# nagadomi/nunif

Hardware: NVIDIA H100
Metric: waifu2x_input_megapixels_per_sec (higher is better)
Workload: dtype f16

## Files before the change

nunif_b200/csrc/swin_attention_mma.cu:

```cuda
#include "common.cuh"
#include "gemm_wgmma.cuh"
#include "swin_kernels.h"
#include "tmap.h"

namespace nb200 {

extern int g_tune[16];

namespace {
constexpr int WS = 6, WTOK = 36, WPAD = 48, HEADS = 6;
constexpr const char* SHIFT_ONE_AXIS_MSG =
    "shifted window attention needs H and W both equal to the 6-token window or both larger (torchvision drops the shift per "
    "axis; these kernels shift both axes or neither)";
}

constexpr int NKT = 5;

template <int D>
struct AttnCtx {
    __half* sq;
    const int* sreg;
    const float4* bf;
    const __half* kbase[NKT];
    const __half* vbase[3];
    int hc, g, t4;
    float scale;
    bool boundary;
};

template <int D, int LD, bool LAST, int BNT = 6>
__device__ __forceinline__ void attn_mtile(const AttnCtx<D>& cx, int mt) {
    constexpr uint32_t ONES = 0x3C003C00u;
    constexpr int HL = LAST ? 1 : 2;
    const int g = cx.g, t4 = cx.t4, hc = cx.hc;
    const int row0 = min(mt * 16 + g, WTOK - 1), row1 = min(mt * 16 + g + 8, WTOK - 1);
    float s[NKT][4];
#pragma unroll
    for (int nt = 0; nt < NKT; ++nt)
#pragma unroll
        for (int r = 0; r < 4; ++r) s[nt][r] = 0.f;
#pragma unroll
    for (int kt = 0; kt < D / 16; ++kt) {
        uint32_t a[4];
        const __half* p0 = cx.sq + row0 * LD + hc + kt * 16 + 2 * t4;
        const __half* p1 = cx.sq + row1 * LD + hc + kt * 16 + 2 * t4;
        a[0] = *reinterpret_cast<const uint32_t*>(p0);
        a[1] = *reinterpret_cast<const uint32_t*>(p1);
        a[2] = *reinterpret_cast<const uint32_t*>(p0 + 8);
        a[3] = *reinterpret_cast<const uint32_t*>(p1 + 8);
#pragma unroll
        for (int nt = 0; nt < NKT; ++nt) {
            const __half* pk = cx.kbase[nt] + kt * 16;
            mma16816(s[nt], a, *reinterpret_cast<const uint32_t*>(pk), *reinterpret_cast<const uint32_t*>(pk + 8));
        }
    }
#pragma unroll
    for (int nt = 0; nt < NKT; ++nt) {
        const float4 bv = BNT == 6 ? __ldg(cx.bf + (mt * 6 + nt) * 32) : cx.bf[(mt * BNT + nt) * 32];
        s[nt][0] = fmaf(s[nt][0], cx.scale, bv.x);
        s[nt][1] = fmaf(s[nt][1], cx.scale, bv.y);
        if (!LAST) {
            s[nt][2] = fmaf(s[nt][2], cx.scale, bv.z);
            s[nt][3] = fmaf(s[nt][3], cx.scale, bv.w);
        }
    }
    if (cx.boundary) {
        const int q0 = cx.sreg[row0], q1 = cx.sreg[row1];
#pragma unroll
        for (int nt = 0; nt < NKT; ++nt)
#pragma unroll
            for (int e = 0; e < 2; ++e) {
                const int cr = cx.sreg[min(nt * 8 + 2 * t4 + e, WTOK - 1)];
                if (cr != q0) s[nt][e] += -100.0f * 1.4426950408889634f;
                if (!LAST && cr != q1) s[nt][2 + e] += -100.0f * 1.4426950408889634f;
            }
    }
#pragma unroll
    for (int hlf = 0; hlf < HL; ++hlf) {
        float mx = -1e30f;
#pragma unroll
        for (int nt = 0; nt < NKT; ++nt) mx = fmaxf(mx, fmaxf(s[nt][2 * hlf], s[nt][2 * hlf + 1]));
        mx = fmaxf(mx, __shfl_xor_sync(0xffffffffu, mx, 1));
        mx = fmaxf(mx, __shfl_xor_sync(0xffffffffu, mx, 2));
#pragma unroll
        for (int nt = 0; nt < NKT; ++nt)
#pragma unroll
            for (int e = 0; e < 2; ++e) {
                s[nt][2 * hlf + e] = ex2(s[nt][2 * hlf + e] - mx);
            }
    }
    if (LAST) {
#pragma unroll
        for (int nt = 0; nt < NKT; ++nt) s[nt][2] = s[nt][3] = 0.f;
    }
    float o[D / 8][4], osum[4] = {0.f, 0.f, 0.f, 0.f};
#pragma unroll
    for (int nt = 0; nt < D / 8; ++nt)
#pragma unroll
        for (int r = 0; r < 4; ++r) o[nt][r] = 0.f;
#pragma unroll
    for (int kt = 0; kt < 2; ++kt) {
        uint32_t a[4];
        a[0] = pack_half2(s[2 * kt][0], s[2 * kt][1]);
        a[1] = pack_half2(s[2 * kt][2], s[2 * kt][3]);
        a[2] = pack_half2(s[2 * kt + 1][0], s[2 * kt + 1][1]);
        a[3] = pack_half2(s[2 * kt + 1][2], s[2 * kt + 1][3]);
        mma16816(osum, a, ONES, ONES);
#pragma unroll
        for (int nt = 0; nt < D / 8; ++nt) {
            uint32_t b[2];
            ldmatrix_x2_trans(b, smem_u32(cx.vbase[kt] + nt * 8));
            mma16816(o[nt], a, b[0], b[1]);
        }
    }
    {
        const uint32_t a0 = pack_half2(s[4][0], s[4][1]), a1 = pack_half2(s[4][2], s[4][3]);
        mma1688(osum, a0, a1, ONES);
#pragma unroll
        for (int nt = 0; nt < D / 8; ++nt) {
            mma1688(o[nt], a0, a1, ldmatrix_x1_trans(smem_u32(cx.vbase[2] + nt * 8)));
        }
    }
    const float inv0 = __fdividef(1.f, osum[0]);
    const float inv1 = LAST ? 0.f : __fdividef(1.f, osum[2]);
    __syncwarp();
    const int r0 = mt * 16 + g, r1 = r0 + 8;
#pragma unroll
    for (int nt = 0; nt < D / 8; ++nt) {
        if (!LAST || r0 < WTOK) *reinterpret_cast<uint32_t*>(cx.sq + r0 * LD + hc + nt * 8 + 2 * t4) = pack_half2(o[nt][0] * inv0, o[nt][1] * inv0);
        if (!LAST) *reinterpret_cast<uint32_t*>(cx.sq + r1 * LD + hc + nt * 8 + 2 * t4) = pack_half2(o[nt][2] * inv1, o[nt][3] * inv1);
    }
}

template <int D>
__global__ void __launch_bounds__(192, D == 16 ? 6 : 4) window_attention_mma_kernel(const __half* __restrict__ qkv, const float4* __restrict__ bias_frag,
                                                                   __half* __restrict__ out, int H, int W, int shift,
                                                                   size_t plane) {
    if (threadIdx.x == 0) NB_PDL_TRIGGER();
    constexpr int C = D * HEADS;
    constexpr int LD = C + 8;
    extern __shared__ __align__(16) unsigned char smem_raw[];
    __half* sq = reinterpret_cast<__half*>(smem_raw);
    __half* sk = sq + WTOK * LD;
    __half* sv = sk + WTOK * LD;
    int* stok = reinterpret_cast<int*>(sv + WTOK * LD);
    int* sreg = stok + WTOK;
    const int nww = W / WS;
    const int wx = blockIdx.x % nww, wy = blockIdx.x / nww, b = blockIdx.y;
    const int tid = threadIdx.x;
    if (tid < WPAD) {
        int reg = -1;
        if (tid < WTOK) {
            const int ry = wy * WS + tid / WS, rx = wx * WS + tid % WS;
            const int y = (ry + shift) % H, x = (rx + shift) % W;
            stok[tid] = (b * H + y) * W + x;
            int hr = 0, wr = 0;
            if (shift > 0) {
                hr = ry < H - WS ? 0 : (ry < H - shift ? 1 : 2);
                wr = rx < W - WS ? 0 : (rx < W - shift ? 1 : 2);
            }
            reg = hr * 3 + wr;
        }
        sreg[tid] = reg;
    }
    __syncthreads();
    constexpr int VPT = C / 8;
    constexpr int RG = 192 / VPT;
    const int vv = tid % VPT, rg = tid / VPT;
    for (int t = rg; t < WTOK; t += RG) {
        const __half* src = qkv + (size_t)stok[t] * C + vv * 8;
        __half* dst = sq + t * LD + vv * 8;
        cp_async16(dst, src);
        cp_async16(dst + WTOK * LD, src + plane);
        cp_async16(dst + 2 * WTOK * LD, src + 2 * plane);
    }
    cp_async_commit();
    cp_async_wait<0>();
    __syncthreads();

    const int head = tid >> 5, lane = tid & 31, g = lane >> 2, t4 = lane & 3;
    const int hc = head * D;
    const float scale = ((D == 16) ? 0.25f : 0.17677669529663687f) * 1.4426950408889634f;
    const bool boundary = shift > 0 && (wy == gridDim.x / nww - 1 || wx == nww - 1);
    const float4* bf = bias_frag + (size_t)head * (3 * 6 * 32) + lane;
    AttnCtx<D> cx;
    cx.sq = sq; cx.sreg = sreg; cx.bf = bf; cx.hc = hc; cx.g = g; cx.t4 = t4; cx.scale = scale; cx.boundary = boundary;
#pragma unroll
    for (int nt = 0; nt < NKT; ++nt) cx.kbase[nt] = sk + min(nt * 8 + g, WTOK - 1) * LD + hc + 2 * t4;
    cx.vbase[0] = sv + (lane & 15) * LD + hc;
    cx.vbase[1] = sv + (16 + (lane & 15)) * LD + hc;
    cx.vbase[2] = sv + min(32 + (lane & 7), WTOK - 1) * LD + hc;
#pragma unroll 1
    for (int mt = 0; mt < 2; ++mt) attn_mtile<D, LD, false>(cx, mt);
    attn_mtile<D, LD, true>(cx, 2);
    __syncthreads();
    for (int t = rg; t < WTOK; t += RG)
        *reinterpret_cast<uint4*>(out + (size_t)stok[t] * C + vv * 8) = *reinterpret_cast<const uint4*>(sq + t * LD + vv * 8);
}

__global__ void build_bias_frag_kernel(const float* __restrict__ table, float4* __restrict__ frag) {
    const int i = blockIdx.x * blockDim.x + threadIdx.x;
    if (i >= HEADS * 3 * 6 * 32) return;
    const int lane = i & 31, nt = (i >> 5) % 6, mt = (i / (32 * 6)) % 3, head = i / (32 * 6 * 3);
    const int g = lane >> 2, t4 = lane & 3;
    float v[4];
#pragma unroll
    for (int r = 0; r < 4; ++r) {
        const int row = mt * 16 + g + 8 * (r >> 1), col = nt * 8 + 2 * t4 + (r & 1);
        if (col >= WTOK) v[r] = -1e30f;
        else if (row >= WTOK) v[r] = 0.f;
        else {
            const int qy = row / WS, qx = row % WS, ky = col / WS, kx = col % WS;
            v[r] = 1.4426950408889634f * table[((qy - ky + WS - 1) * (2 * WS - 1) + (qx - kx + WS - 1)) * HEADS + head];
        }
    }
    frag[i] = make_float4(v[0], v[1], v[2], v[3]);
}

int build_bias_frag(cudaStream_t st, const float* table, float* frag) {
    build_bias_frag_kernel<<<(HEADS * 3 * 6 * 32 + 255) / 256, 256, 0, st>>>(table, reinterpret_cast<float4*>(frag));
    NB_LAUNCHED();
    return 0;
}

template <int D>
static size_t attn_smem_bytes() {
    constexpr int C = D * HEADS, LD = C + 8;
    return (size_t)3 * WTOK * LD * 2 + (WTOK + WPAD) * 4 + 16;
}

static int check_window_geometry(const char* func, bool fused, int H, int W, int C, int* shift) {
    auto refuse = [&](const std::string& msg) { return fail(std::string(func) + ": " + msg); };
    if (H % WS != 0 || W % WS != 0) return refuse("feature map must be a multiple of the 6x6 window");
    if (C != 96 && C != 192) return refuse(std::string(fused ? "fused " : "") + "window attention supports C=96 (d=16) and C=192 (d=32)");
    if (*shift != 0 && (H == WS) != (W == WS)) return refuse(SHIFT_ONE_AXIS_MSG);
    if (WS >= H) *shift = 0;
    return 0;
}

int window_attention(cudaStream_t st, const __half* qkv, const float* bias_frag_f, __half* out, int B, int H, int W, int C,
                     int shift, size_t plane) {
    const float4* bias_table = reinterpret_cast<const float4*>(bias_frag_f);
    if (check_window_geometry(__func__, false, H, W, C, &shift)) return 1;
    dim3 grid((H / WS) * (W / WS), B);
    ProfScope ps(st, PC_ATTN, (double)B * H * W * C * 4 * 2, (double)B * H * W * C * 3 * 2, (double)B * H * W * C * 2);
    if (C == 96) {
        const int want = g_tune[6] > 0 ? g_tune[6] : 72;
        if (ensure_dyn_smem((const void*)window_attention_mma_kernel<16>, attn_smem_bytes<16>(), want)) return 1;
        window_attention_mma_kernel<16><<<grid, 192, attn_smem_bytes<16>(), st>>>(qkv, bias_table, out, H, W, shift, plane);
    } else {
        const int want = g_tune[6] > 0 ? g_tune[6] : 86;
        if (ensure_dyn_smem((const void*)window_attention_mma_kernel<32>, attn_smem_bytes<32>(), want)) return 1;
        window_attention_mma_kernel<32><<<grid, 192, attn_smem_bytes<32>(), st>>>(qkv, bias_table, out, H, W, shift, plane);
    }
    NB_LAUNCHED();
    return 0;
}


constexpr int FA_ROWS = 128, FA_WIN = 3, FA_SLOT = 96 * 64, FA_KPS = 3, FA_STAGES = 4;
constexpr int FA_MMA_THREADS = GEMM_CONSUMER_THREADS, FA_PRODUCER_WARP = FA_MMA_THREADS / 32, FA_ATTN_WARPS = 11;
constexpr int FA_THREADS = FA_MMA_THREADS + 32 + 32 * FA_ATTN_WARPS;
constexpr int FA_LD = 32 + 8;
constexpr int FA_CHUNK_BYTES = FA_WIN * 3 * WTOK * FA_LD * 2;
constexpr int FA_STAGE = FA_KPS * FA_SLOT;

template <int C>
struct FaCfg {
    static constexpr int X_BYTES = FA_ROWS * C * 2;
    static constexpr bool SBF = C == 96;
    static constexpr int SBF_BYTES = SBF ? HEADS * 3 * NKT * 32 * 16 : 0;
    static constexpr int SBF_OFF = 2 * X_BYTES + FA_STAGES * FA_STAGE + 2 * FA_CHUNK_BYTES + 4 * WPAD * 4 + (2 * FA_STAGES + 8) * 8 +
                                   3 * C * 4;
    static constexpr int SMEM = SBF_OFF + SBF_BYTES + 1024;
    static_assert(SBF_OFF % 16 == 0, "float4 bias fragments");
    static_assert(SMEM <= 232448, "over the 227 KB opt-in shared memory of an H100 CTA");
};

__device__ __forceinline__ int fa_token(int b, int wy, int wx, int t, int H, int W, int shift) {
    int y = wy * WS + t / WS + shift, xx = wx * WS + t % WS + shift;
    if (y >= H) y -= H;
    if (xx >= W) xx -= W;
    return (b * H + y) * W + xx;
}

template <int C>
__global__ void __launch_bounds__(FA_THREADS, 1) swin_attn_fused_kernel(const __grid_constant__ CUtensorMap wmap,
                                                                        const __half* __restrict__ x, const float* __restrict__ bqkv,
                                                                        const float4* __restrict__ bias_frag, __half* __restrict__ out,
                                                                        int H, int W, int shift, int nwin) {
    using Cfg = FaCfg<C>;
    constexpr int D = C / HEADS, KB = C / 32, NCH = C / 32, HPC = 32 / D;
    constexpr int IPC = 3 * FA_WIN * HPC, IPT = NCH * IPC;
    constexpr int SPC = KB / FA_KPS;
    constexpr int VPR = C / 8;
    static_assert(KB % FA_KPS == 0, "a ring stage holds FA_KPS K-blocks of one chunk");
    static_assert(FA_WIN == 3, "the gather selects among 3 windows");
    extern __shared__ uint8_t smem_dyn[];
    uint8_t* smem = smem_dyn + ((1024u - (smem_u32(smem_dyn) & 1023u)) & 1023u);
    uint8_t* sx = smem;
    uint8_t* ring = smem + 2 * Cfg::X_BYTES;
    __half* schunk = reinterpret_cast<__half*>(ring + FA_STAGES * FA_STAGE);
    int* sreg = reinterpret_cast<int*>(reinterpret_cast<uint8_t*>(schunk) + 2 * FA_CHUNK_BYTES);
    uint64_t* full = reinterpret_cast<uint64_t*>(sreg + 4 * WPAD);
    uint64_t* empty = full + FA_STAGES;
    uint64_t* afull = empty + FA_STAGES;
    uint64_t* aempty = afull + 2;
    uint64_t* cfull = aempty + 2;
    uint64_t* cempty = cfull + 2;
    float* sbias = reinterpret_cast<float*>(cempty + 2);
    float4* sbf = reinterpret_cast<float4*>(smem + Cfg::SBF_OFF);
    const int tid = threadIdx.x, warp = tid >> 5, lane = tid & 31;
    const int nww = W / WS, nwy = H / WS;
    const int ntiles = (nwin + FA_WIN - 1) / FA_WIN;
    const int ntl = (ntiles - (int)blockIdx.x + (int)gridDim.x - 1) / (int)gridDim.x;

    if (tid < 4 * WPAD) {
        const int p = tid / WPAD, t = tid % WPAD;
        int reg = -1;
        if (t < WTOK) {
            const int hr = (p & 2) ? (t / WS < WS - shift ? 1 : 2) : 0;
            const int wr = (p & 1) ? (t % WS < WS - shift ? 1 : 2) : 0;
            reg = hr * 3 + wr;
        }
        sreg[tid] = reg;
    }
    for (int i = tid; i < 3 * C; i += FA_THREADS) sbias[i] = bqkv[i];
    if (Cfg::SBF)
        for (int i = tid; i < HEADS * 3 * NKT * 32; i += FA_THREADS)
            sbf[i] = __ldg(bias_frag + ((i >> 5) / NKT * 6 + (i >> 5) % NKT) * 32 + (i & 31));
    for (int i = tid; i < 2 * (FA_ROWS - FA_WIN * WTOK) * VPR; i += FA_THREADS) {
        const int bsel = i / ((FA_ROWS - FA_WIN * WTOK) * VPR), j = i % ((FA_ROWS - FA_WIN * WTOK) * VPR);
        const int r = FA_WIN * WTOK + j / VPR, u = j % VPR;
        *reinterpret_cast<uint4*>(sx + bsel * Cfg::X_BYTES + (u >> 2) * (FA_ROWS * 64) + stage_off<32>(r, u & 3)) =
            make_uint4(0u, 0u, 0u, 0u);
    }
    if (tid == FA_MMA_THREADS) {
        tma_prefetch_desc(&wmap);
        for (int s = 0; s < FA_STAGES; ++s) {
            mbar_init(&full[s], 1);
            mbar_init(&empty[s], 2);
        }
        for (int b = 0; b < 2; ++b) {
            mbar_init(&afull[b], 32 * FA_ATTN_WARPS);
            mbar_init(&aempty[b], 2);
            mbar_init(&cfull[b], FA_MMA_THREADS / 32);
            mbar_init(&cempty[b], IPC);
        }
        fence_barrier_init();
    }
    fence_async_smem();
    __syncthreads();
    if (tid == 0) NB_PDL_TRIGGER();

    if (warp == FA_PRODUCER_WARP) {
        if (elect_one()) {
            int q = 0;
#pragma unroll 1
            for (int k = 0; k < ntl; ++k) {
#pragma unroll 1
                for (int i = 0; i < NCH * SPC; ++i, ++q) {
                    const int s = q % FA_STAGES, c = i / SPC, kb0 = (i % SPC) * FA_KPS;
                    mbar_wait(&empty[s], ((q / FA_STAGES) & 1) ^ 1);
                    mbar_expect_tx(&full[s], FA_STAGE);
#pragma unroll
                    for (int kk = 0; kk < FA_KPS; ++kk)
#pragma unroll
                        for (int m = 0; m < 3; ++m)
                            tma_load_2d(&wmap, &full[s], ring + s * FA_STAGE + kk * FA_SLOT + m * 32 * 64, (kb0 + kk) * 32, m * C + 32 * c);
                }
            }
        }
        return;
    }

    const float scale = ((D == 16) ? 0.25f : 0.17677669529663687f) * 1.4426950408889634f;
    const int g = lane >> 2, t4 = lane & 3;
    if (warp > FA_PRODUCER_WARP) {
        const int aw = warp - FA_PRODUCER_WARP - 1;
        auto gather = [&](int tile, uint8_t* sa) {
            int wb[FA_WIN], wwy[FA_WIN], wwx[FA_WIN];
#pragma unroll
            for (int w = 0; w < FA_WIN; ++w) {
                const int gw = tile * FA_WIN + w, b = gw / (nww * nwy), rw = gw - b * (nww * nwy);
                wb[w] = gw < nwin ? b : -1;
                wwy[w] = rw / nww;
                wwx[w] = rw - wwy[w] * nww;
            }
            for (int i = aw * 32 + lane; i < FA_WIN * WTOK * VPR; i += 32 * FA_ATTN_WARPS) {
                const int r = i / VPR, u = i % VPR, w = r / WTOK;
                const int b = w == 0 ? wb[0] : (w == 1 ? wb[1] : wb[2]);
                const int wy = w == 0 ? wwy[0] : (w == 1 ? wwy[1] : wwy[2]), wx = w == 0 ? wwx[0] : (w == 1 ? wwx[1] : wwx[2]);
                uint8_t* dst = sa + (u >> 2) * (FA_ROWS * 64) + stage_off<32>(r, u & 3);
                if (b >= 0) cp_async16(dst, x + (size_t)fa_token(b, wy, wx, r - w * WTOK, H, W, shift) * C + u * 8);
                else *reinterpret_cast<uint4*>(dst) = make_uint4(0u, 0u, 0u, 0u);
            }
            cp_async_commit();
        };
        auto gathered = [&](int kt) {
            cp_async_wait<0>();
            fence_async_smem();
            mbar_arrive(&afull[kt & 1]);
        };
        gather(blockIdx.x, sx);
        gathered(0);
        int kcur = -1, nth = 0;
#pragma unroll 1
        for (int n = aw; n < ntl * IPT; n += FA_ATTN_WARPS) {
            const int gc = n / IPC, item = n - gc * IPC, c = gc % NCH;
            const int kt = n / IPT, tile = blockIdx.x + kt * gridDim.x;
            mbar_wait(&cfull[gc & 1], (gc >> 1) & 1);
            if (kt != kcur) {
                kcur = kt;
                nth = 0;
            }
            if (kt + 1 < ntl && nth == 0) {
                mbar_wait(&aempty[(kt + 1) & 1], (((kt + 1) >> 1) & 1) ^ 1);
                gather(tile + gridDim.x, sx + ((kt + 1) & 1) * Cfg::X_BYTES);
            }
            if (kt + 1 < ntl && nth == 1) gathered(kt + 1);
            ++nth;
            const int mt = item / (FA_WIN * HPC), pr = item - mt * (FA_WIN * HPC), w = pr / HPC, hh = pr - w * HPC;
            const int gw = tile * FA_WIN + w;
            if (gw < nwin) {
                const int b = gw / (nww * nwy), r = gw % (nww * nwy), wy = r / nww, wx = r % nww, head = c * HPC + hh;
                const bool lrow = wy == nwy - 1, lcol = wx == nww - 1;
                __half* sq = schunk + (gc & 1) * (FA_CHUNK_BYTES / 2) + w * 3 * WTOK * FA_LD;
                __half* sk = sq + WTOK * FA_LD;
                __half* sv = sk + WTOK * FA_LD;
                AttnCtx<D> cx;
                cx.sq = sq; cx.sreg = sreg + (2 * lrow + lcol) * WPAD;
                cx.bf = Cfg::SBF ? sbf + head * (3 * NKT * 32) + lane : bias_frag + (size_t)head * (3 * 6 * 32) + lane;
                cx.hc = hh * D; cx.g = g; cx.t4 = t4; cx.scale = scale;
                cx.boundary = shift > 0 && (lrow || lcol);
#pragma unroll
                for (int nt = 0; nt < NKT; ++nt) cx.kbase[nt] = sk + min(nt * 8 + g, WTOK - 1) * FA_LD + cx.hc + 2 * t4;
                cx.vbase[0] = sv + (lane & 15) * FA_LD + cx.hc;
                cx.vbase[1] = sv + (16 + (lane & 15)) * FA_LD + cx.hc;
                cx.vbase[2] = sv + min(32 + (lane & 7), WTOK - 1) * FA_LD + cx.hc;
                constexpr int BNT = Cfg::SBF ? NKT : 6;
                if (mt < 2) attn_mtile<D, FA_LD, false, BNT>(cx, mt);
                else attn_mtile<D, FA_LD, true, BNT>(cx, 2);
                __syncwarp();
                const int nrow = mt < 2 ? 16 : WTOK - 32;
                for (int e = lane; e < nrow * (D / 8); e += 32) {
                    const int tk = 16 * mt + e / (D / 8), u = e % (D / 8);
                    *reinterpret_cast<uint4*>(out + (size_t)fa_token(b, wy, wx, tk, H, W, shift) * C + head * D + u * 8) =
                        *reinterpret_cast<const uint4*>(sq + tk * FA_LD + cx.hc + u * 8);
                }
            }
            __syncwarp();
            if (lane == 0) mbar_arrive(&cempty[gc & 1]);
        }
        return;
    }

    const int wg = tid >> 7, t = tid & 127;
    const int row0 = wg * 64 + (t >> 5) * 16 + ((t & 31) >> 2);
    const int cq = 2 * (t & 3);
    int q = 0, gc = 0;
#pragma unroll 1
    for (int k = 0; k < ntl; ++k) {
        mbar_wait(&afull[k & 1], (k >> 1) & 1);
        const uint32_t a_base = smem_u32(sx + (k & 1) * Cfg::X_BYTES) + wg * 64 * 64;
#pragma unroll 1
        for (int c = 0; c < NCH; ++c, ++gc) {
            float acc[48];
#pragma unroll
            for (int j = 0; j < 48; ++j) acc[j] = 0.f;
#pragma unroll 1
            for (int j = 0; j < SPC; ++j, ++q) {
                const int s = q % FA_STAGES;
                mbar_wait(&full[s], (q / FA_STAGES) & 1);
                wgmma_fence();
#pragma unroll
                for (int kk = 0; kk < FA_KPS; ++kk) {
                    const uint32_t a = a_base + (j * FA_KPS + kk) * (FA_ROWS * 64), bb = smem_u32(ring + s * FA_STAGE + kk * FA_SLOT);
                    wgmma_f16<96>(acc, make_kmajor_desc<64>(a), make_kmajor_desc<64>(bb), 1u);
                    wgmma_f16<96>(acc, make_kmajor_desc<64>(a + 32), make_kmajor_desc<64>(bb + 32), 1u);
                }
                wgmma_commit();
                wgmma_wait<1>();
                if (j > 0 && t == 0) mbar_arrive(&empty[(q - 1) % FA_STAGES]);
            }
            wgmma_wait<0>();
            if (t == 0) {
                mbar_arrive(&empty[(q - 1) % FA_STAGES]);
                if (c == NCH - 1) mbar_arrive(&aempty[k & 1]);
            }
            wgmma_fence_operands(acc);
            mbar_wait(&cempty[gc & 1], ((gc >> 1) & 1) ^ 1);
            __half* sqkv = schunk + (gc & 1) * (FA_CHUNK_BYTES / 2);
#pragma unroll
            for (int j = 0; j < 12; ++j) {
                const int m = j >> 2, col = 8 * (j & 3) + cq;
                const float2 bq = *reinterpret_cast<const float2*>(sbias + m * C + 32 * c + col);
#pragma unroll
                for (int i = 0; i < 2; ++i) {
                    const int r = row0 + 8 * i;
                    if (r < FA_WIN * WTOK) {
                        const int w = r / WTOK, tk = r - w * WTOK;
                        *reinterpret_cast<__half2*>(sqkv + ((w * 3 + m) * WTOK + tk) * FA_LD + col) =
                            __floats2half2_rn(acc[4 * j + 2 * i] + bq.x, acc[4 * j + 2 * i + 1] + bq.y);
                    }
                }
            }
            __syncwarp();
            if (lane == 0) mbar_arrive(&cfull[gc & 1]);
        }
    }
}

int swin_attn_fused(cudaStream_t st, const __half* x, const __half* wqkv, const float* bqkv, const float* bias_frag_f, __half* att,
                    int B, int H, int W, int C, int shift) {
    NB_CHECK(x && wqkv && bqkv && bias_frag_f && att, "null pointer");
    if (check_window_geometry(__func__, true, H, W, C, &shift)) return 1;
    const long long nwin = (long long)B * (H / WS) * (W / WS);
    NB_CHECK(nwin > 0 && nwin < (1LL << 31), "window count out of range");
    CUtensorMap wmap;
    const cuuint64_t dims[2] = {(cuuint64_t)C, (cuuint64_t)(3 * C)};
    const cuuint64_t strides[1] = {(cuuint64_t)C * 2};
    const cuuint32_t box[2] = {32, 32};
    if (encode(&wmap, wqkv, 2, dims, strides, box, 64)) return 1;
    const double T = (double)B * H * W;
    ProfScope ps(st, PC_FUSED_ATTN, T * 3.0 * C * C * 2 + T * C * 36 * 4, T * C * 2, T * C * 2);
    const long long ntiles = (nwin + FA_WIN - 1) / FA_WIN;
    long long grid = std::min<long long>(ntiles, device_sm_count());
    if (g_tune[11] > 0) grid = std::min<long long>(grid, g_tune[11]);
    if (rec_on()) rec_launch("swin_attn", {{"B", B}, {"H", H}, {"W", W}, {"C", C}, {"shift", shift}});
    const float4* bf = reinterpret_cast<const float4*>(bias_frag_f);
    if (C == 96) {
        if (ensure_dyn_smem((const void*)swin_attn_fused_kernel<96>, FaCfg<96>::SMEM)) return 1;
        swin_attn_fused_kernel<96><<<(unsigned)grid, FA_THREADS, FaCfg<96>::SMEM, st>>>(wmap, x, bqkv, bf, att, H, W, shift, (int)nwin);
    } else {
        if (ensure_dyn_smem((const void*)swin_attn_fused_kernel<192>, FaCfg<192>::SMEM)) return 1;
        swin_attn_fused_kernel<192><<<(unsigned)grid, FA_THREADS, FaCfg<192>::SMEM, st>>>(wmap, x, bqkv, bf, att, H, W, shift, (int)nwin);
    }
    NB_LAUNCHED();
    return 0;
}

template <typename F>
static int with_bias_frag(void* stream, const float* table, F call) {
    cudaStream_t st = (cudaStream_t)stream;
    float* frag = nullptr;
    NB_CUDA(cudaMallocAsync((void**)&frag, BIAS_FRAG_FLOATS * sizeof(float), st));
    int rc = build_bias_frag(st, table, frag);
    if (!rc) rc = call(st, frag);
    cudaFreeAsync(frag, st);
    return rc;
}

}

using namespace nb200;

extern "C" int nb200_window_attention_f16(const void* qkv, const float* bias_table, void* out, int B, int H, int W, int C,
                                          int heads, int shift, void* stream) {
    NB_CHECK(qkv && bias_table && out, "null pointer");
    NB_CHECK(heads == 6, "only 6 heads are supported");
    return with_bias_frag(stream, bias_table, [&](cudaStream_t st, const float* frag) {
        return window_attention(st, (const __half*)qkv, frag, (__half*)out, B, H, W, C, shift, (size_t)B * H * W * C);
    });
}

extern "C" int nb200_swin_attn_fused_f16(const void* x, const void* wqkv, const float* bqkv, const float* bias_table, void* att,
                                         int B, int H, int W, int C, int shift, void* stream) {
    NB_CHECK(bias_table, "null pointer");
    return with_bias_frag(stream, bias_table, [&](cudaStream_t st, const float* frag) {
        return swin_attn_fused(st, (const __half*)x, (const __half*)wqkv, bqkv, frag, (__half*)att, B, H, W, C, shift);
    });
}
```

Measured before the change: 81.25.

## Process all heads of a chunk per attention item and deepen chunk/gather pipelining

The attention mtile helper now handles several heads per call (NH), so one warp item covers every head of a 32-channel chunk instead of one head. This cuts per-item overhead and lets each item store full 64-byte rows. The fused attention kernel adds a configurable number of QKV chunk buffers (three for C=96, with ring stages reduced to three) and prefetches input tiles two ahead rather than one. The gather for tile k+2 is issued by the warps handling the tail of tile k. The cost is more registers per warp and a more intricate mbarrier parity scheme, which could hurt occupancy or risk deadlock if the static assumptions fail.

```diff
diff --git a/nunif_b200/csrc/swin_attention_mma.cu b/nunif_b200/csrc/swin_attention_mma.cu
--- a/nunif_b200/csrc/swin_attention_mma.cu
+++ b/nunif_b200/csrc/swin_attention_mma.cu
@@ -28,42 +28,49 @@
     bool boundary;
 };
 
-template <int D, int LD, bool LAST, int BNT = 6>
+template <int D, int LD, bool LAST, int BNT = 6, int NH = 1>
 __device__ __forceinline__ void attn_mtile(const AttnCtx<D>& cx, int mt) {
     constexpr uint32_t ONES = 0x3C003C00u;
     constexpr int HL = LAST ? 1 : 2;
+    constexpr int HBF = 3 * BNT * 32;
     const int g = cx.g, t4 = cx.t4, hc = cx.hc;
     const int row0 = min(mt * 16 + g, WTOK - 1), row1 = min(mt * 16 + g + 8, WTOK - 1);
-    float s[NKT][4];
-#pragma unroll
-    for (int nt = 0; nt < NKT; ++nt)
-#pragma unroll
-        for (int r = 0; r < 4; ++r) s[nt][r] = 0.f;
-#pragma unroll
-    for (int kt = 0; kt < D / 16; ++kt) {
-        uint32_t a[4];
-        const __half* p0 = cx.sq + row0 * LD + hc + kt * 16 + 2 * t4;
-        const __half* p1 = cx.sq + row1 * LD + hc + kt * 16 + 2 * t4;
-        a[0] = *reinterpret_cast<const uint32_t*>(p0);
-        a[1] = *reinterpret_cast<const uint32_t*>(p1);
-        a[2] = *reinterpret_cast<const uint32_t*>(p0 + 8);
-        a[3] = *reinterpret_cast<const uint32_t*>(p1 + 8);
+    float s[NH][NKT][4];
+#pragma unroll
+    for (int h = 0; h < NH; ++h)
+#pragma unroll
+        for (int nt = 0; nt < NKT; ++nt)
+#pragma unroll
+            for (int r = 0; r < 4; ++r) s[h][nt][r] = 0.f;
+#pragma unroll
+    for (int h = 0; h < NH; ++h)
+#pragma unroll
+        for (int kt = 0; kt < D / 16; ++kt) {
+            uint32_t a[4];
+            const __half* p0 = cx.sq + row0 * LD + hc + h * D + kt * 16 + 2 * t4;
+            const __half* p1 = cx.sq + row1 * LD + hc + h * D + kt * 16 + 2 * t4;
+            a[0] = *reinterpret_cast<const uint32_t*>(p0);
+            a[1] = *reinterpret_cast<const uint32_t*>(p1);
+            a[2] = *reinterpret_cast<const uint32_t*>(p0 + 8);
+            a[3] = *reinterpret_cast<const uint32_t*>(p1 + 8);
+#pragma unroll
+            for (int nt = 0; nt < NKT; ++nt) {
+                const __half* pk = cx.kbase[nt] + h * D + kt * 16;
+                mma16816(s[h][nt], a, *reinterpret_cast<const uint32_t*>(pk), *reinterpret_cast<const uint32_t*>(pk + 8));
+            }
+        }
+#pragma unroll
+    for (int h = 0; h < NH; ++h)
 #pragma unroll
         for (int nt = 0; nt < NKT; ++nt) {
-            const __half* pk = cx.kbase[nt] + kt * 16;
-            mma16816(s[nt], a, *reinterpret_cast<const uint32_t*>(pk), *reinterpret_cast<const uint32_t*>(pk + 8));
-        }
-    }
-#pragma unroll
-    for (int nt = 0; nt < NKT; ++nt) {
-        const float4 bv = BNT == 6 ? __ldg(cx.bf + (mt * 6 + nt) * 32) : cx.bf[(mt * BNT + nt) * 32];
-        s[nt][0] = fmaf(s[nt][0], cx.scale, bv.x);
-        s[nt][1] = fmaf(s[nt][1], cx.scale, bv.y);
-        if (!LAST) {
-            s[nt][2] = fmaf(s[nt][2], cx.scale, bv.z);
-            s[nt][3] = fmaf(s[nt][3], cx.scale, bv.w);
-        }
-    }
+            const float4 bv = BNT == 6 ? __ldg(cx.bf + h * HBF + (mt * 6 + nt) * 32) : cx.bf[h * HBF + (mt * BNT + nt) * 32];
+            s[h][nt][0] = fmaf(s[h][nt][0], cx.scale, bv.x);
+            s[h][nt][1] = fmaf(s[h][nt][1], cx.scale, bv.y);
+            if (!LAST) {
+                s[h][nt][2] = fmaf(s[h][nt][2], cx.scale, bv.z);
+                s[h][nt][3] = fmaf(s[h][nt][3], cx.scale, bv.w);
+            }
+        }
     if (cx.boundary) {
         const int q0 = cx.sreg[row0], q1 = cx.sreg[row1];
 #pragma unroll
@@ -71,64 +78,75 @@
 #pragma unroll
             for (int e = 0; e < 2; ++e) {
                 const int cr = cx.sreg[min(nt * 8 + 2 * t4 + e, WTOK - 1)];
-                if (cr != q0) s[nt][e] += -100.0f * 1.4426950408889634f;
-                if (!LAST && cr != q1) s[nt][2 + e] += -100.0f * 1.4426950408889634f;
-            }
-    }
-#pragma unroll
-    for (int hlf = 0; hlf < HL; ++hlf) {
-        float mx = -1e30f;
-#pragma unroll
-        for (int nt = 0; nt < NKT; ++nt) mx = fmaxf(mx, fmaxf(s[nt][2 * hlf], s[nt][2 * hlf + 1]));
-        mx = fmaxf(mx, __shfl_xor_sync(0xffffffffu, mx, 1));
-        mx = fmaxf(mx, __shfl_xor_sync(0xffffffffu, mx, 2));
-#pragma unroll
-        for (int nt = 0; nt < NKT; ++nt)
-#pragma unroll
-            for (int e = 0; e < 2; ++e) {
-                s[nt][2 * hlf + e] = ex2(s[nt][2 * hlf + e] - mx);
-            }
-    }
-    if (LAST) {
-#pragma unroll
-        for (int nt = 0; nt < NKT; ++nt) s[nt][2] = s[nt][3] = 0.f;
-    }
-    float o[D / 8][4], osum[4] = {0.f, 0.f, 0.f, 0.f};
-#pragma unroll
-    for (int nt = 0; nt < D / 8; ++nt)
-#pragma unroll
-        for (int r = 0; r < 4; ++r) o[nt][r] = 0.f;
-#pragma unroll
-    for (int kt = 0; kt < 2; ++kt) {
-        uint32_t a[4];
-        a[0] = pack_half2(s[2 * kt][0], s[2 * kt][1]);
-        a[1] = pack_half2(s[2 * kt][2], s[2 * kt][3]);
-        a[2] = pack_half2(s[2 * kt + 1][0], s[2 * kt + 1][1]);
-        a[3] = pack_half2(s[2 * kt + 1][2], s[2 * kt + 1][3]);
-        mma16816(osum, a, ONES, ONES);
+#pragma unroll
+                for (int h = 0; h < NH; ++h) {
+                    if (cr != q0) s[h][nt][e] += -100.0f * 1.4426950408889634f;
+                    if (!LAST && cr != q1) s[h][nt][2 + e] += -100.0f * 1.4426950408889634f;
+                }
+            }
+    }
+    uint32_t p[NH][NKT][2];
+#pragma unroll
+    for (int h = 0; h < NH; ++h) {
+#pragma unroll
+        for (int hlf = 0; hlf < HL; ++hlf) {
+            float mx = -1e30f;
+#pragma unroll
+            for (int nt = 0; nt < NKT; ++nt) mx = fmaxf(mx, fmaxf(s[h][nt][2 * hlf], s[h][nt][2 * hlf + 1]));
+            mx = fmaxf(mx, __shfl_xor_sync(0xffffffffu, mx, 1));
+            mx = fmaxf(mx, __shfl_xor_sync(0xffffffffu, mx, 2));
+#pragma unroll
+            for (int nt = 0; nt < NKT; ++nt)
+                p[h][nt][hlf] = pack_half2(ex2(s[h][nt][2 * hlf] - mx), ex2(s[h][nt][2 * hlf + 1] - mx));
+        }
+        if (LAST) {
+#pragma unroll
+            for (int nt = 0; nt < NKT; ++nt) p[h][nt][1] = pack_half2(0.f, 0.f);
+        }
+    }
+    float o[NH][D / 8][4], osum[NH][4];
+#pragma unroll
+    for (int h = 0; h < NH; ++h) {
+#pragma unroll
+        for (int r = 0; r < 4; ++r) osum[h][r] = 0.f;
+#pragma unroll
+        for (int nt = 0; nt < D / 8; ++nt)
+#pragma unroll
+            for (int r = 0; r < 4; ++r) o[h][nt][r] = 0.f;
+    }
+#pragma unroll
+    for (int kt = 0; kt < 2; ++kt)
+#pragma unroll
+        for (int h = 0; h < NH; ++h) {
+            const uint32_t a[4] = {p[h][2 * kt][0], p[h][2 * kt][1], p[h][2 * kt + 1][0], p[h][2 * kt + 1][1]};
+            mma16816(osum[h], a, ONES, ONES);
+#pragma unroll
+            for (int nt = 0; nt < D / 8; ++nt) {
+                uint32_t b[2];
+                ldmatrix_x2_trans(b, smem_u32(cx.vbase[kt] + h * D + nt * 8));
+                mma16816(o[h][nt], a, b[0], b[1]);
+            }
+        }
+#pragma unroll
+    for (int h = 0; h < NH; ++h) {
+        mma1688(osum[h], p[h][4][0], p[h][4][1], ONES);
 #pragma unroll
         for (int nt = 0; nt < D / 8; ++nt) {
-            uint32_t b[2];
-            ldmatrix_x2_trans(b, smem_u32(cx.vbase[kt] + nt * 8));
-            mma16816(o[nt], a, b[0], b[1]);
-        }
-    }
-    {
-        const uint32_t a0 = pack_half2(s[4][0], s[4][1]), a1 = pack_half2(s[4][2], s[4][3]);
-        mma1688(osum, a0, a1, ONES);
-#pragma unroll
-        for (int nt = 0; nt < D / 8; ++nt) {
-            mma1688(o[nt], a0, a1, ldmatrix_x1_trans(smem_u32(cx.vbase[2] + nt * 8)));
-        }
-    }
-    const float inv0 = __fdividef(1.f, osum[0]);
-    const float inv1 = LAST ? 0.f : __fdividef(1.f, osum[2]);
+            mma1688(o[h][nt], p[h][4][0], p[h][4][1], ldmatrix_x1_trans(smem_u32(cx.vbase[2] + h * D + nt * 8)));
+        }
+    }
     __syncwarp();
     const int r0 = mt * 16 + g, r1 = r0 + 8;
 #pragma unroll
-    for (int nt = 0; nt < D / 8; ++nt) {
-        if (!LAST || r0 < WTOK) *reinterpret_cast<uint32_t*>(cx.sq + r0 * LD + hc + nt * 8 + 2 * t4) = pack_half2(o[nt][0] * inv0, o[nt][1] * inv0);
-        if (!LAST) *reinterpret_cast<uint32_t*>(cx.sq + r1 * LD + hc + nt * 8 + 2 * t4) = pack_half2(o[nt][2] * inv1, o[nt][3] * inv1);
+    for (int h = 0; h < NH; ++h) {
+        const float inv0 = __fdividef(1.f, osum[h][0]);
+        const float inv1 = LAST ? 0.f : __fdividef(1.f, osum[h][2]);
+#pragma unroll
+        for (int nt = 0; nt < D / 8; ++nt) {
+            __half* dst = cx.sq + hc + h * D + nt * 8 + 2 * t4;
+            if (!LAST || r0 < WTOK) *reinterpret_cast<uint32_t*>(dst + r0 * LD) = pack_half2(o[h][nt][0] * inv0, o[h][nt][1] * inv0);
+            if (!LAST) *reinterpret_cast<uint32_t*>(dst + r1 * LD) = pack_half2(o[h][nt][2] * inv1, o[h][nt][3] * inv1);
+        }
     }
 }
 
@@ -258,7 +276,7 @@
 }
 
 
-constexpr int FA_ROWS = 128, FA_WIN = 3, FA_SLOT = 96 * 64, FA_KPS = 3, FA_STAGES = 4;
+constexpr int FA_ROWS = 128, FA_WIN = 3, FA_SLOT = 96 * 64, FA_KPS = 3;
 constexpr int FA_MMA_THREADS = GEMM_CONSUMER_THREADS, FA_PRODUCER_WARP = FA_MMA_THREADS / 32, FA_ATTN_WARPS = 11;
 constexpr int FA_THREADS = FA_MMA_THREADS + 32 + 32 * FA_ATTN_WARPS;
 constexpr int FA_LD = 32 + 8;
@@ -270,8 +288,9 @@
     static constexpr int X_BYTES = FA_ROWS * C * 2;
     static constexpr bool SBF = C == 96;
     static constexpr int SBF_BYTES = SBF ? HEADS * 3 * NKT * 32 * 16 : 0;
-    static constexpr int SBF_OFF = 2 * X_BYTES + FA_STAGES * FA_STAGE + 2 * FA_CHUNK_BYTES + 4 * WPAD * 4 + (2 * FA_STAGES + 8) * 8 +
-                                   3 * C * 4;
+    static constexpr int STAGES = C == 96 ? 3 : 4, NCB = C == 96 ? 3 : 2;
+    static constexpr int SBF_OFF = 2 * X_BYTES + STAGES * FA_STAGE + NCB * FA_CHUNK_BYTES + 4 * WPAD * 4 +
+                                   (2 * STAGES + 4 + 2 * NCB) * 8 + 3 * C * 4;
     static constexpr int SMEM = SBF_OFF + SBF_BYTES + 1024;
     static_assert(SBF_OFF % 16 == 0, "float4 bias fragments");
     static_assert(SMEM <= 232448, "over the 227 KB opt-in shared memory of an H100 CTA");
@@ -291,24 +310,27 @@
                                                                         int H, int W, int shift, int nwin) {
     using Cfg = FaCfg<C>;
     constexpr int D = C / HEADS, KB = C / 32, NCH = C / 32, HPC = 32 / D;
-    constexpr int IPC = 3 * FA_WIN * HPC, IPT = NCH * IPC;
+    constexpr int IPC = 3 * FA_WIN, IPT = NCH * IPC;
     constexpr int SPC = KB / FA_KPS;
     constexpr int VPR = C / 8;
     static_assert(KB % FA_KPS == 0, "a ring stage holds FA_KPS K-blocks of one chunk");
-    static_assert(FA_WIN == 3, "the gather selects among 3 windows");
+    static_assert(FA_WIN == 3, "the gather and the items select among 3 windows");
+    static_assert(IPT >= FA_ATTN_WARPS, "every attention warp gathers and signals tile k + 2 at its last item of tile k");
+    static_assert(FA_ATTN_WARPS <= 2 * IPC, "a warp's consecutive items are at most 2 chunks apart (cfull parity waits)");
     extern __shared__ uint8_t smem_dyn[];
     uint8_t* smem = smem_dyn + ((1024u - (smem_u32(smem_dyn) & 1023u)) & 1023u);
     uint8_t* sx = smem;
     uint8_t* ring = smem + 2 * Cfg::X_BYTES;
-    __half* schunk = reinterpret_cast<__half*>(ring + FA_STAGES * FA_STAGE);
-    int* sreg = reinterpret_cast<int*>(reinterpret_cast<uint8_t*>(schunk) + 2 * FA_CHUNK_BYTES);
+    constexpr int STAGES = Cfg::STAGES, NCB = Cfg::NCB;
+    __half* schunk = reinterpret_cast<__half*>(ring + STAGES * FA_STAGE);
+    int* sreg = reinterpret_cast<int*>(reinterpret_cast<uint8_t*>(schunk) + NCB * FA_CHUNK_BYTES);
     uint64_t* full = reinterpret_cast<uint64_t*>(sreg + 4 * WPAD);
-    uint64_t* empty = full + FA_STAGES;
-    uint64_t* afull = empty + FA_STAGES;
+    uint64_t* empty = full + STAGES;
+    uint64_t* afull = empty + STAGES;
     uint64_t* aempty = afull + 2;
     uint64_t* cfull = aempty + 2;
-    uint64_t* cempty = cfull + 2;
-    float* sbias = reinterpret_cast<float*>(cempty + 2);
+    uint64_t* cempty = cfull + NCB;
+    float* sbias = reinterpret_cast<float*>(cempty + NCB);
     float4* sbf = reinterpret_cast<float4*>(smem + Cfg::SBF_OFF);
     const int tid = threadIdx.x, warp = tid >> 5, lane = tid & 31;
     const int nww = W / WS, nwy = H / WS;
@@ -337,13 +359,15 @@
     }
     if (tid == FA_MMA_THREADS) {
         tma_prefetch_desc(&wmap);
-        for (int s = 0; s < FA_STAGES; ++s) {
+        for (int s = 0; s < STAGES; ++s) {
             mbar_init(&full[s], 1);
             mbar_init(&empty[s], 2);
         }
         for (int b = 0; b < 2; ++b) {
             mbar_init(&afull[b], 32 * FA_ATTN_WARPS);
             mbar_init(&aempty[b], 2);
+        }
+        for (int b = 0; b < NCB; ++b) {
             mbar_init(&cfull[b], FA_MMA_THREADS / 32);
             mbar_init(&cempty[b], IPC);
         }
@@ -360,8 +384,8 @@
             for (int k = 0; k < ntl; ++k) {
 #pragma unroll 1
                 for (int i = 0; i < NCH * SPC; ++i, ++q) {
-                    const int s = q % FA_STAGES, c = i / SPC, kb0 = (i % SPC) * FA_KPS;
-                    mbar_wait(&empty[s], ((q / FA_STAGES) & 1) ^ 1);
+                    const int s = q % STAGES, c = i / SPC, kb0 = (i % SPC) * FA_KPS;
+                    mbar_wait(&empty[s], ((q / STAGES) & 1) ^ 1);
                     mbar_expect_tx(&full[s], FA_STAGE);
 #pragma unroll
                     for (int kk = 0; kk < FA_KPS; ++kk)
@@ -378,8 +402,7 @@
     const int g = lane >> 2, t4 = lane & 3;
     if (warp > FA_PRODUCER_WARP) {
         const int aw = warp - FA_PRODUCER_WARP - 1;
-        auto gather = [&](int tile, uint8_t* sa) {
-            int wb[FA_WIN], wwy[FA_WIN], wwx[FA_WIN];
+        auto windows = [&](int tile, int (&wb)[FA_WIN], int (&wwy)[FA_WIN], int (&wwx)[FA_WIN]) {
 #pragma unroll
             for (int w = 0; w < FA_WIN; ++w) {
                 const int gw = tile * FA_WIN + w, b = gw / (nww * nwy), rw = gw - b * (nww * nwy);
@@ -387,6 +410,10 @@
                 wwy[w] = rw / nww;
                 wwx[w] = rw - wwy[w] * nww;
             }
+        };
+        auto gather = [&](int tile, uint8_t* sa) {
+            int wb[FA_WIN], wwy[FA_WIN], wwx[FA_WIN];
+            windows(tile, wb, wwy, wwx);
             for (int i = aw * 32 + lane; i < FA_WIN * WTOK * VPR; i += 32 * FA_ATTN_WARPS) {
                 const int r = i / VPR, u = i % VPR, w = r / WTOK;
                 const int b = w == 0 ? wb[0] : (w == 1 ? wb[1] : wb[2]);
@@ -403,54 +430,58 @@
             mbar_arrive(&afull[kt & 1]);
         };
         gather(blockIdx.x, sx);
+        if (ntl > 1) gather(blockIdx.x + gridDim.x, sx + Cfg::X_BYTES);
         gathered(0);
-        int kcur = -1, nth = 0;
+        if (ntl > 1) gathered(1);
+        int kcur = -1;
+        int wb[FA_WIN], wwy[FA_WIN], wwx[FA_WIN];
 #pragma unroll 1
         for (int n = aw; n < ntl * IPT; n += FA_ATTN_WARPS) {
             const int gc = n / IPC, item = n - gc * IPC, c = gc % NCH;
             const int kt = n / IPT, tile = blockIdx.x + kt * gridDim.x;
-            mbar_wait(&cfull[gc & 1], (gc >> 1) & 1);
+            mbar_wait(&cfull[gc % NCB], (gc / NCB) & 1);
             if (kt != kcur) {
                 kcur = kt;
-                nth = 0;
-            }
-            if (kt + 1 < ntl && nth == 0) {
-                mbar_wait(&aempty[(kt + 1) & 1], (((kt + 1) >> 1) & 1) ^ 1);
-                gather(tile + gridDim.x, sx + ((kt + 1) & 1) * Cfg::X_BYTES);
-            }
-            if (kt + 1 < ntl && nth == 1) gathered(kt + 1);
-            ++nth;
-            const int mt = item / (FA_WIN * HPC), pr = item - mt * (FA_WIN * HPC), w = pr / HPC, hh = pr - w * HPC;
-            const int gw = tile * FA_WIN + w;
-            if (gw < nwin) {
-                const int b = gw / (nww * nwy), r = gw % (nww * nwy), wy = r / nww, wx = r % nww, head = c * HPC + hh;
+                windows(tile, wb, wwy, wwx);
+            }
+            const int j = kt + 2;
+            const bool gathering = j < ntl && n + FA_ATTN_WARPS >= (kt + 1) * IPT;
+            if (gathering) {
+                mbar_wait(&aempty[j & 1], ((j >> 1) & 1) ^ 1);
+                gather(tile + 2 * gridDim.x, sx + (j & 1) * Cfg::X_BYTES);
+            }
+            const int mt = item / FA_WIN, w = item - mt * FA_WIN;
+            const int b = w == 0 ? wb[0] : (w == 1 ? wb[1] : wb[2]);
+            if (b >= 0) {
+                const int wy = w == 0 ? wwy[0] : (w == 1 ? wwy[1] : wwy[2]), wx = w == 0 ? wwx[0] : (w == 1 ? wwx[1] : wwx[2]);
                 const bool lrow = wy == nwy - 1, lcol = wx == nww - 1;
-                __half* sq = schunk + (gc & 1) * (FA_CHUNK_BYTES / 2) + w * 3 * WTOK * FA_LD;
+                __half* sq = schunk + (gc % NCB) * (FA_CHUNK_BYTES / 2) + w * 3 * WTOK * FA_LD;
                 __half* sk = sq + WTOK * FA_LD;
                 __half* sv = sk + WTOK * FA_LD;
                 AttnCtx<D> cx;
                 cx.sq = sq; cx.sreg = sreg + (2 * lrow + lcol) * WPAD;
-                cx.bf = Cfg::SBF ? sbf + head * (3 * NKT * 32) + lane : bias_frag + (size_t)head * (3 * 6 * 32) + lane;
-                cx.hc = hh * D; cx.g = g; cx.t4 = t4; cx.scale = scale;
+                cx.bf = Cfg::SBF ? sbf + c * HPC * (3 * NKT * 32) + lane : bias_frag + (size_t)c * HPC * (3 * 6 * 32) + lane;
+                cx.hc = 0; cx.g = g; cx.t4 = t4; cx.scale = scale;
                 cx.boundary = shift > 0 && (lrow || lcol);
 #pragma unroll
-                for (int nt = 0; nt < NKT; ++nt) cx.kbase[nt] = sk + min(nt * 8 + g, WTOK - 1) * FA_LD + cx.hc + 2 * t4;
-                cx.vbase[0] = sv + (lane & 15) * FA_LD + cx.hc;
-                cx.vbase[1] = sv + (16 + (lane & 15)) * FA_LD + cx.hc;
-                cx.vbase[2] = sv + min(32 + (lane & 7), WTOK - 1) * FA_LD + cx.hc;
+                for (int nt = 0; nt < NKT; ++nt) cx.kbase[nt] = sk + min(nt * 8 + g, WTOK - 1) * FA_LD + 2 * t4;
+                cx.vbase[0] = sv + (lane & 15) * FA_LD;
+                cx.vbase[1] = sv + (16 + (lane & 15)) * FA_LD;
+                cx.vbase[2] = sv + min(32 + (lane & 7), WTOK - 1) * FA_LD;
                 constexpr int BNT = Cfg::SBF ? NKT : 6;
-                if (mt < 2) attn_mtile<D, FA_LD, false, BNT>(cx, mt);
-                else attn_mtile<D, FA_LD, true, BNT>(cx, 2);
+                if (mt < 2) attn_mtile<D, FA_LD, false, BNT, HPC>(cx, mt);
+                else attn_mtile<D, FA_LD, true, BNT, HPC>(cx, 2);
                 __syncwarp();
                 const int nrow = mt < 2 ? 16 : WTOK - 32;
-                for (int e = lane; e < nrow * (D / 8); e += 32) {
-                    const int tk = 16 * mt + e / (D / 8), u = e % (D / 8);
-                    *reinterpret_cast<uint4*>(out + (size_t)fa_token(b, wy, wx, tk, H, W, shift) * C + head * D + u * 8) =
-                        *reinterpret_cast<const uint4*>(sq + tk * FA_LD + cx.hc + u * 8);
+                for (int e = lane; e < nrow * 4; e += 32) {
+                    const int tk = 16 * mt + (e >> 2), u = e & 3;
+                    *reinterpret_cast<uint4*>(out + (size_t)fa_token(b, wy, wx, tk, H, W, shift) * C + 32 * c + u * 8) =
+                        *reinterpret_cast<const uint4*>(sq + tk * FA_LD + u * 8);
                 }
             }
             __syncwarp();
-            if (lane == 0) mbar_arrive(&cempty[gc & 1]);
+            if (lane == 0) mbar_arrive(&cempty[gc % NCB]);
+            if (gathering) gathered(j);
         }
         return;
     }
@@ -470,8 +501,8 @@
             for (int j = 0; j < 48; ++j) acc[j] = 0.f;
 #pragma unroll 1
             for (int j = 0; j < SPC; ++j, ++q) {
-                const int s = q % FA_STAGES;
-                mbar_wait(&full[s], (q / FA_STAGES) & 1);
+                const int s = q % STAGES;
+                mbar_wait(&full[s], (q / STAGES) & 1);
                 wgmma_fence();
 #pragma unroll
                 for (int kk = 0; kk < FA_KPS; ++kk) {
@@ -481,16 +512,16 @@
                 }
                 wgmma_commit();
                 wgmma_wait<1>();
-                if (j > 0 && t == 0) mbar_arrive(&empty[(q - 1) % FA_STAGES]);
+                if (j > 0 && t == 0) mbar_arrive(&empty[(q - 1) % STAGES]);
             }
             wgmma_wait<0>();
             if (t == 0) {
-                mbar_arrive(&empty[(q - 1) % FA_STAGES]);
+                mbar_arrive(&empty[(q - 1) % STAGES]);
                 if (c == NCH - 1) mbar_arrive(&aempty[k & 1]);
             }
             wgmma_fence_operands(acc);
-            mbar_wait(&cempty[gc & 1], ((gc >> 1) & 1) ^ 1);
-            __half* sqkv = schunk + (gc & 1) * (FA_CHUNK_BYTES / 2);
+            mbar_wait(&cempty[gc % NCB], ((gc / NCB) & 1) ^ 1);
+            __half* sqkv = schunk + (gc % NCB) * (FA_CHUNK_BYTES / 2);
 #pragma unroll
             for (int j = 0; j < 12; ++j) {
                 const int m = j >> 2, col = 8 * (j & 3) + cq;
@@ -506,7 +537,7 @@
                 }
             }
             __syncwarp();
-            if (lane == 0) mbar_arrive(&cfull[gc & 1]);
+            if (lane == 0) mbar_arrive(&cfull[gc % NCB]);
         }
     }
 }
```

New measurement: 82.84, median of 6. 2.0% higher.
